# hpcaitech/Open-Sora

Measured on NVIDIA H100. Metric: denoise-steps/sec STDiT3-XL/2 64x32x32 bf16, higher is better.
Workload: dtype bf16

## Files before the change

### open-sora_b200/csrc/attn_sm90.cu

```cuda
#include <stdlib.h>

#include "common.cuh"
#include "stage.cuh"
#include "tiles.cuh"

namespace osb {

constexpr int kAttnThreads = 256;
constexpr int kKeyBlock = 64;

template <int D>
struct FlashState {
  static constexpr int DP = HeadTileCfg<D>::DP;
  uint32_t q[DP / 16][4];
  float o[DP / 8][4];
  float m[2], l[2];
};

template <int D>
__device__ __forceinline__ void flash_load_q(FlashState<D>& f, uint32_t sq, uint32_t chunk_bytes) {
  using Cfg = HeadTileCfg<D>;
  const int lane = threadIdx.x & 31, warp = threadIdx.x >> 5;
  const int row = warp * 16 + (lane & 15);
#pragma unroll
  for (int kk = 0; kk < Cfg::DP / 16; ++kk)
    ldsm_x4(sq + tile_unit_off<Cfg::MAIN>(row, 2 * kk + (lane >> 4), chunk_bytes), f.q[kk][0], f.q[kk][1], f.q[kk][2], f.q[kk][3]);
#pragma unroll
  for (int j = 0; j < Cfg::DP / 8; ++j) f.o[j][0] = f.o[j][1] = f.o[j][2] = f.o[j][3] = 0.f;
  f.m[0] = f.m[1] = -INFINITY;
  f.l[0] = f.l[1] = 0.f;
}

template <int D, bool kBias = false>
__device__ __forceinline__ void flash_block(FlashState<D>& f, uint32_t sk, uint32_t sv, uint32_t chunk_bytes, int krow0,
                                            int n16, int key0, const int (&lo)[2], const int (&hi)[2], float sc,
                                            const float* bias = nullptr, int boff0 = 0, int boff1 = 0, float bscale = 0.f) {
  using Cfg = HeadTileCfg<D>;
  constexpr int NB = kKeyBlock / 8;
  const int lane = threadIdx.x & 31;
  float s[NB][4];
#pragma unroll
  for (int g = 0; g < kKeyBlock / 16; ++g) {
    s[2 * g][0] = s[2 * g][1] = s[2 * g][2] = s[2 * g][3] = 0.f;
    s[2 * g + 1][0] = s[2 * g + 1][1] = s[2 * g + 1][2] = s[2 * g + 1][3] = 0.f;
    if (g >= n16) continue;
    const int krow = krow0 + g * 16 + (lane & 7) + ((lane >> 4) << 3);
#pragma unroll
    for (int kk = 0; kk < Cfg::DP / 16; ++kk) {
      uint32_t b0, b1, b2, b3;
      ldsm_x4(sk + tile_unit_off<Cfg::MAIN>(krow, 2 * kk + ((lane >> 3) & 1), chunk_bytes), b0, b1, b2, b3);
      mma_bf16_16816(s[2 * g], f.q[kk], b0, b1);
      mma_bf16_16816(s[2 * g + 1], f.q[kk], b2, b3);
    }
  }
  float mx[2] = {-INFINITY, -INFINITY};
#pragma unroll
  for (int j = 0; j < NB; ++j) {
// ... 19 lines not shown
  }
#pragma unroll
  for (int j = 0; j < Cfg::DP / 8; ++j) {
    f.o[j][0] *= alpha[0]; f.o[j][1] *= alpha[0];
    f.o[j][2] *= alpha[1]; f.o[j][3] *= alpha[1];
  }
#pragma unroll
  for (int j = 0; j < NB; ++j) {
#pragma unroll
    for (int e = 0; e < 4; ++e) {
      s[j][e] = fast_exp2(fmaf(s[j][e], sc, -ms[e >> 1]));
      f.l[e >> 1] += s[j][e];
    }
  }
#pragma unroll
  for (int g = 0; g < kKeyBlock / 16; ++g) {
    if (g >= n16) continue;
    const uint32_t a[4] = {pack_bf16x2(s[2 * g][0], s[2 * g][1]), pack_bf16x2(s[2 * g][2], s[2 * g][3]),
                           pack_bf16x2(s[2 * g + 1][0], s[2 * g + 1][1]), pack_bf16x2(s[2 * g + 1][2], s[2 * g + 1][3])};
    const int vrow = krow0 + g * 16 + (lane & 7) + (((lane >> 3) & 1) << 3);
#pragma unroll
    for (int dg = 0; dg < Cfg::DP / 16; ++dg) {
      uint32_t b0, b1, b2, b3;
      ldsm_x4_t(sv + tile_unit_off<Cfg::MAIN>(vrow, 2 * dg + (lane >> 4), chunk_bytes), b0, b1, b2, b3);
      mma_bf16_16816(f.o[2 * dg], a, b0, b1);
      mma_bf16_16816(f.o[2 * dg + 1], a, b2, b3);
    }
  }
}

template <int D>
__device__ __forceinline__ void flash_store(FlashState<D>& f, __nv_bfloat16* dst0, __nv_bfloat16* dst1) {
  const int lane = threadIdx.x & 31;
  float inv[2];
#pragma unroll
  for (int i = 0; i < 2; ++i) {
    float l = f.l[i];
    l += __shfl_xor_sync(0xffffffffu, l, 1);
    l += __shfl_xor_sync(0xffffffffu, l, 2);
    inv[i] = l > 0.f ? 1.0f / l : 0.f;
  }
#pragma unroll
  for (int j = 0; j < D / 8; ++j) {
    const int c = 8 * j + 2 * (lane & 3);
    if (dst0) *reinterpret_cast<uint32_t*>(dst0 + c) = pack_bf16x2(f.o[j][0] * inv[0], f.o[j][1] * inv[0]);
    if (dst1) *reinterpret_cast<uint32_t*>(dst1 + c) = pack_bf16x2(f.o[j][2] * inv[1], f.o[j][3] * inv[1]);
  }
}

struct TileAttnParams {
  const uint8_t* q; const uint8_t* k; const uint8_t* v;
  int64_t q_head_stride, kv_head_stride;
  TileMap qmap;
  int32_t q_tile_bytes, q_slot_bytes;
  int32_t kv_tile_bytes, kv_slot_bytes;
  int32_t BK, nkb, Lk;
  int64_t num_seqs, num_sets;
  const int32_t* kv_lens;
  __nv_bfloat16* out;
  int64_t out_ld;
  float scale_log2;
  RowScatter out_sc;
};

template <int D>
__global__ void __launch_bounds__(kAttnThreads, 1) attn_tiles_kernel(const TileAttnParams p) {
  extern __shared__ __align__(1024) uint8_t smem[];
  const uint32_t s0 = smem_u32(smem);
  const uint32_t sQ = s0;
  auto sK = [&](int st) { return s0 + (uint32_t)(p.q_slot_bytes + st * 2 * p.kv_slot_bytes); };
  auto sV = [&](int st) { return sK(st) + (uint32_t)p.kv_slot_bytes; };
  const uint32_t bar = s0 + (uint32_t)(p.q_slot_bytes + 4 * p.kv_slot_bytes);
  const uint32_t q_full = bar;
  auto kv_full = [&](int st) { return bar + 8u + 8u * st; };

  const int tid = threadIdx.x, lane = tid & 31, warp = tid >> 5;
  const int64_t qtile = blockIdx.x;
  const int head = blockIdx.y;
  const int64_t set = qtile / p.qmap.tps;
  const int qt = (int)(qtile - set * p.qmap.tps);

  int keys = p.qmap.G > 1 ? p.qmap.G * p.Lk : p.Lk;
  if (p.qmap.G == 1 && p.kv_lens) { const int l = __ldg(p.kv_lens + set); keys = l < keys ? (l < 0 ? 0 : l) : keys; }
  const int nkt = (keys + p.BK - 1) / p.BK;

  if (tid == 0) {
    mbar_init(q_full, 1);
    mbar_init(kv_full(0), 1);
    mbar_init(kv_full(1), 1);
    fence_barrier_init();
  }
  __syncthreads();
  pdl_wait();
  const uint8_t* kbase = p.k + (int64_t)head * p.kv_head_stride + set * p.nkb * (int64_t)p.kv_tile_bytes;
  const uint8_t* vbase = p.v + (int64_t)head * p.kv_head_stride + set * p.nkb * (int64_t)p.kv_tile_bytes;
  if (tid == 0) {
    mbar_expect_tx(q_full, (uint32_t)p.q_tile_bytes);
    bulk_load_1d(sQ, p.q + (int64_t)head * p.q_head_stride + qtile * p.q_tile_bytes, (uint32_t)p.q_tile_bytes, q_full);
    for (int st = 0; st < 2 && st < nkt; ++st) {
      mbar_expect_tx(kv_full(st), 2u * (uint32_t)p.kv_tile_bytes);
      bulk_load_1d(sK(st), kbase + (int64_t)st * p.kv_tile_bytes, (uint32_t)p.kv_tile_bytes, kv_full(st));
      bulk_load_1d(sV(st), vbase + (int64_t)st * p.kv_tile_bytes, (uint32_t)p.kv_tile_bytes, kv_full(st));
    }
  }

  int64_t seq[2];
  int pos[2], lo[2], hi[2];
  bool valid[2];
#pragma unroll
  for (int i = 0; i < 2; ++i) {
    const int r = warp * 16 + (lane >> 2) + 8 * i;
    lo[i] = hi[i] = 0;
    if (p.qmap.G > 1) {
      const int g = r / p.qmap.L;
      pos[i] = r - g * p.qmap.L;
      seq[i] = set * p.qmap.G + g;
      valid[i] = g < p.qmap.G && seq[i] < p.num_seqs;
      if (valid[i]) { lo[i] = g * p.Lk; hi[i] = lo[i] + p.Lk; }
    } else {
      pos[i] = qt * p.qmap.TR + r;
      seq[i] = set;
      valid[i] = r < p.qmap.TR && pos[i] < p.qmap.L;
      if (valid[i]) hi[i] = keys;
    }
  }

  FlashState<D> f;
  mbar_wait(q_full, 0);
  flash_load_q<D>(f, sQ, (uint32_t)p.qmap.TR * 128u);
  const float sc = p.scale_log2;
  for (int kb = 0; kb < nkt; ++kb) {
    const int st = kb & 1;
    mbar_wait(kv_full(st), (uint32_t)(kb >> 1) & 1u);
    for (int k0 = 0; k0 < p.BK; k0 += kKeyBlock) {
      int n = keys - (kb * p.BK + k0);
      const int cap = p.BK - k0 < kKeyBlock ? p.BK - k0 : kKeyBlock;
      n = n > cap ? cap : n;
      if (n <= 0) break;
      const int lo_b[2] = {lo[0], lo[1]}, hi_b[2] = {hi[0], hi[1]};
      flash_block<D>(f, sK(st), sV(st), (uint32_t)p.BK * 128u, k0, (n + 15) >> 4, kb * p.BK + k0, lo_b, hi_b, sc);
    }
    __syncthreads();
    if (tid == 0 && kb + 2 < nkt) {
      mbar_expect_tx(kv_full(st), 2u * (uint32_t)p.kv_tile_bytes);
      bulk_load_1d(sK(st), kbase + (int64_t)(kb + 2) * p.kv_tile_bytes, (uint32_t)p.kv_tile_bytes, kv_full(st));
      bulk_load_1d(sV(st), vbase + (int64_t)(kb + 2) * p.kv_tile_bytes, (uint32_t)p.kv_tile_bytes, kv_full(st));
    }
  }
  pdl_launch_dependents();

  __nv_bfloat16* dst[2] = {nullptr, nullptr};
#pragma unroll
  for (int i = 0; i < 2; ++i) {
    if (!valid[i]) continue;
    int64_t orow = row_of_token(p.qmap, seq[i], pos[i]);
    __nv_bfloat16* obase = p.out;
    if (p.out_sc.mode != 0) {
      int peer;
      scatter_row(p.out_sc, orow, peer, orow);
      obase = static_cast<__nv_bfloat16*>(scatter_base(p.out_sc, peer));
    }
    dst[i] = obase + orow * p.out_ld + (int64_t)head * D;
  }
  flash_store<D>(f, dst[0], dst[1]);
}

template <int D>
static int attn_tiles_launch(TileAttnParams& p, int H, cudaStream_t stream) {
  using Cfg = HeadTileCfg<D>;
  p.q_tile_bytes = p.qmap.TR * Cfg::ROW_BYTES;
  p.q_slot_bytes = 128 * Cfg::ROW_BYTES;
  p.kv_tile_bytes = p.BK * Cfg::ROW_BYTES;
  p.kv_slot_bytes = (p.kv_tile_bytes + 127) / 128 * 128;
  const int smem = p.q_slot_bytes + 4 * p.kv_slot_bytes + 64;
  const int64_t qtiles = p.num_sets * p.qmap.tps;
  if (qtiles >= (1ll << 31) || H > 65535) { set_error("osb_attn_tiles: problem too large (%lld query tiles)", (long long)qtiles); return OSB_ERR_UNSUPPORTED; }
  cudaLaunchAttribute attr[2];
  cudaLaunchConfig_t cfg = launch_config(dim3((unsigned)qtiles, (unsigned)H), dim3(kAttnThreads), smem, stream, attr);
  OSB_CHECK_CUDA(cudaLaunchKernelEx(&cfg, attn_tiles_kernel<D>, p));
  count_launch();
  return OSB_OK;
}

struct AttnParams {
  const __nv_bfloat16* q; const __nv_bfloat16* k; const __nv_bfloat16* v; __nv_bfloat16* out;
  int64_t q_ld, k_ld, v_ld, out_ld;
  int64_t num_seqs, seqs_per_batch;
  int64_t q_bs, q_ss, q_ts, k_bs, k_ss, k_ts;
  int32_t Lq, Lk;
  const int32_t* kv_lens;
  const __nv_bfloat16* qw; const __nv_bfloat16* kw;
  const __nv_bfloat16* qw2; const __nv_bfloat16* kw2;
  int32_t norm_split;
  float eps;
  const float* cos; const float* sin;
  int32_t rope_half;
  float scale_log2;
  int32_t G;
  int32_t tiles_per_seq;
  const float* bias;
  int64_t bias_hs;
  float scale;
};

template <int D>
__device__ __forceinline__ void stage_row(uint4 (&raw)[HeadTileCfg<D>::U], bool norm, float eps, const __nv_bfloat16* w,
                                          const float* cosr, const float* sinr, bool rope_half, uint8_t* tile,
                                          uint32_t chunk_bytes, int row) {
  using Cfg = HeadTileCfg<D>;
  constexpr int U = Cfg::U;
  norm_rope_row<D, U>(raw, norm, eps, w, cosr, sinr, rope_half);
#pragma unroll
  for (int u = 0; u < Cfg::UP; ++u)
    *reinterpret_cast<uint4*>(tile + tile_unit_off<Cfg::MAIN>(row, u, chunk_bytes)) = u < U ? raw[u] : make_uint4(0, 0, 0, 0);
}

template <int D, bool kBias>
__global__ void __launch_bounds__(kAttnThreads, 1) attn_short_kernel(const AttnParams p) {
  using Cfg = HeadTileCfg<D>;
  constexpr int U = Cfg::U;
  extern __shared__ __align__(1024) uint8_t smem[];
  uint8_t* sQ = smem;
  uint8_t* sK = smem + 128 * Cfg::ROW_BYTES;
  uint8_t* sV = sK + kKeyBlock * Cfg::ROW_BYTES;
  const int tid = threadIdx.x, lane = tid & 31, warp = tid >> 5;
  const int64_t unit = blockIdx.x;
  const int h = blockIdx.y;

  int64_t seq0;
  int qt = 0;
  if (p.G > 1) seq0 = unit * p.G;
// ... 71 lines not shown
      const int slot = k0 + s;
      const int kg = slot / p.Lk, ktok = slot - kg * p.Lk;
      const int64_t kseq = seq0 + kg;
      const bool ok = slot < nkeys && kseq < p.num_seqs;
      int64_t krow = 0;
      if (ok) krow = row_of(kseq, ktok, p.k_bs, p.k_ss, p.k_ts);
      uint4 t[U];
      {
        const uint4* ks = reinterpret_cast<const uint4*>(p.k + krow * p.k_ld + (int64_t)h * D);
#pragma unroll
        for (int u = 0; u < U; ++u) t[u] = ok ? __ldg(ks + u) : make_uint4(0, 0, 0, 0);
        const __nv_bfloat16* w = (p.kw2 != nullptr && ktok >= p.norm_split) ? p.kw2 : p.kw;
        const bool rope = ok && p.cos != nullptr;
        stage_row<D>(t, ok && p.kw != nullptr, p.eps, w, rope ? p.cos + (int64_t)ktok * (D / 2) : nullptr,
                     rope ? p.sin + (int64_t)ktok * (D / 2) : nullptr, p.rope_half, sK, kKeyBlock * 128u, s);
      }
      {
        const uint4* vs = reinterpret_cast<const uint4*>(p.v + krow * p.v_ld + (int64_t)h * D);
#pragma unroll
        for (int u = 0; u < U; ++u) t[u] = ok ? __ldg(vs + u) : make_uint4(0, 0, 0, 0);
        stage_row<D>(t, false, 0.f, nullptr, nullptr, nullptr, false, sV, kKeyBlock * 128u, s);
      }
    }
    __syncthreads();
    const int n = nkeys - k0 < kKeyBlock ? nkeys - k0 : kKeyBlock;
    if constexpr (kBias)
      flash_block<D, true>(f, smem_u32(sK), smem_u32(sV), kKeyBlock * 128u, 0, (n + 15) >> 4, k0, lo, hi, sc, bh, boff[0],
                           boff[1], p.scale);
    else
      flash_block<D>(f, smem_u32(sK), smem_u32(sV), kKeyBlock * 128u, 0, (n + 15) >> 4, k0, lo, hi, sc);
    __syncthreads();
  }
  pdl_launch_dependents();
  flash_store<D>(f, dst[0], dst[1]);
}

template <int D, bool kBias = false>
static int attn_short_launch(const AttnParams& p, int64_t units, int H, cudaStream_t stream) {
  using Cfg = HeadTileCfg<D>;
  const int smem = (128 + 2 * kKeyBlock) * Cfg::ROW_BYTES;
  cudaLaunchAttribute attr[2];
  cudaLaunchConfig_t cfg = launch_config(dim3((unsigned)units, (unsigned)H), dim3(kAttnThreads), smem, stream, attr);
  OSB_CHECK_CUDA(cudaLaunchKernelEx(&cfg, attn_short_kernel<D, kBias>, p));
  count_launch();
  return OSB_OK;
}

int attn_init() {
  constexpr int kMax = 200 * 1024;
  OSB_CHECK_CUDA(cudaFuncSetAttribute(attn_short_kernel<64, false>, cudaFuncAttributeMaxDynamicSharedMemorySize, kMax));
  OSB_CHECK_CUDA(cudaFuncSetAttribute(attn_short_kernel<72, false>, cudaFuncAttributeMaxDynamicSharedMemorySize, kMax));
  OSB_CHECK_CUDA(cudaFuncSetAttribute(attn_short_kernel<128, false>, cudaFuncAttributeMaxDynamicSharedMemorySize, kMax));
  OSB_CHECK_CUDA(cudaFuncSetAttribute(attn_short_kernel<64, true>, cudaFuncAttributeMaxDynamicSharedMemorySize, kMax));
  OSB_CHECK_CUDA(cudaFuncSetAttribute(attn_tiles_kernel<64>, cudaFuncAttributeMaxDynamicSharedMemorySize, kMax));
  OSB_CHECK_CUDA(cudaFuncSetAttribute(attn_tiles_kernel<72>, cudaFuncAttributeMaxDynamicSharedMemorySize, kMax));
  OSB_CHECK_CUDA(cudaFuncSetAttribute(attn_tiles_kernel<128>, cudaFuncAttributeMaxDynamicSharedMemorySize, kMax));
  return OSB_OK;
}

}

extern "C" int64_t osb_head_tiles_per_head(const osb_tile_map* m, int64_t rows) {
  if (m == nullptr || m->L <= 0 || m->tile_rows <= 0) return -1;
  const int64_t seqs = rows / m->L;
  if (m->G > 1) return (seqs + m->G - 1) / m->G;
  return seqs * m->tps;
}

extern "C" int osb_attn_tiles(const osb_attn_tiles_args* a, void* stream) {
  using namespace osb;
  if (!initialised()) { set_error("osb_init() has not been called"); return OSB_ERR_NOT_INIT; }
  OSB_REQUIRE(a != nullptr, "osb_attn_tiles: null args");
  OSB_REQUIRE(a->q_tiles && a->k_tiles && a->v_tiles && (a->out || a->out_scatter), "osb_attn_tiles: null tensor");
  const int D = a->head_dim;
  OSB_REQUIRE(D == 64 || D == 72 || D == 128, "osb_attn_tiles: head_dim %d not built (64, 72, 128)", D);
  const osb_tile_map& m = a->q_map;
  OSB_REQUIRE(m.mode == 0 || m.mode == 1, "osb_attn_tiles: unknown tile map mode %d", m.mode);
  OSB_REQUIRE(m.L > 0 && m.G >= 1 && m.tile_rows > 0 && m.tile_rows <= 128 && m.tile_rows % 8 == 0,
              "osb_attn_tiles: bad q tile map (L %d G %d rows %d)", m.L, m.G, m.tile_rows);
  OSB_REQUIRE(m.G == 1 ? (m.tps == (m.L + m.tile_rows - 1) / m.tile_rows) : (m.G * m.L <= m.tile_rows && m.tps == 1),
              "osb_attn_tiles: q tile map inconsistent (L %d G %d tps %d rows %d)", m.L, m.G, m.tps, m.tile_rows);
  OSB_REQUIRE(m.mode == 0 || (m.S > 0 && m.T == m.L), "osb_attn_tiles: temporal map needs S > 0 and T == L");
  OSB_REQUIRE(a->kv_tile_rows >= 16 && a->kv_tile_rows <= 128 && a->kv_tile_rows % 16 == 0,
              "osb_attn_tiles: key tiles must have 16..128 rows in multiples of 16, got %d", a->kv_tile_rows);
  OSB_REQUIRE(a->Lk > 0 && a->kv_tiles_per_set >= 1 && (int64_t)a->kv_tiles_per_set * a->kv_tile_rows >= (int64_t)(m.G > 1 ? m.G : 1) * a->Lk,
              "osb_attn_tiles: %d key tiles of %d rows cannot hold %d keys", a->kv_tiles_per_set, a->kv_tile_rows, a->Lk);
  OSB_REQUIRE(m.G == 1 || (a->kv_tiles_per_set == 1), "osb_attn_tiles: packed sequences use one key tile per set");
  OSB_REQUIRE(a->num_seqs > 0 && a->num_heads > 0, "osb_attn_tiles: empty problem");
  OSB_REQUIRE(a->out_ld % 8 == 0 && (reinterpret_cast<uintptr_t>(a->out) & 15) == 0, "osb_attn_tiles: out must be 16-byte aligned");
  OSB_REQUIRE(((reinterpret_cast<uintptr_t>(a->q_tiles) | reinterpret_cast<uintptr_t>(a->k_tiles) | reinterpret_cast<uintptr_t>(a->v_tiles)) & 15) == 0 &&
              a->q_head_stride % 16 == 0 && a->kv_head_stride % 16 == 0, "osb_attn_tiles: tile buffers must be 16-byte aligned");

  TileAttnParams p = {};
  p.q = static_cast<const uint8_t*>(a->q_tiles);
  p.k = static_cast<const uint8_t*>(a->k_tiles);
  p.v = static_cast<const uint8_t*>(a->v_tiles);
  p.q_head_stride = a->q_head_stride; p.kv_head_stride = a->kv_head_stride;
  p.qmap.mode = m.mode; p.qmap.L = m.L; p.qmap.S = m.S; p.qmap.T = m.T; p.qmap.G = m.G; p.qmap.tps = m.tps; p.qmap.TR = m.tile_rows;
  p.BK = a->kv_tile_rows; p.nkb = a->kv_tiles_per_set; p.Lk = a->Lk;
  p.num_seqs = a->num_seqs;
  p.num_sets = m.G > 1 ? (a->num_seqs + m.G - 1) / m.G : a->num_seqs;
  p.kv_lens = a->kv_lens;
  p.out = static_cast<__nv_bfloat16*>(a->out);
  p.out_ld = a->out_ld;
  p.scale_log2 = a->softmax_scale * 1.4426950408889634f;
  {
    const int64_t out_rows = a->num_seqs * m.L;
    const int rc = make_row_scatter(&p.out_sc, a->out_scatter, out_rows, "osb_attn_tiles");
    if (rc) return rc;
// ... 83 lines not shown
```

### open-sora_b200/csrc/wgmma.cuh

```cuda
#pragma once

#include <stdint.h>

namespace osb {

template <int N>
struct Wgmma;

template <>
struct Wgmma<64> {
  static constexpr int kRegs = 32;
  __device__ __forceinline__ static void mma(float (&d)[32], uint64_t da, uint64_t db, uint32_t accumulate) {
    asm volatile(
        "{\n\t.reg .pred p;\n\tsetp.ne.b32 p, %34, 0;\n\t"
        "wgmma.mma_async.sync.aligned.m64n64k16.f32.bf16.bf16 "
        "{%0, %1, %2, %3, %4, %5, %6, %7, %8, %9, %10, %11, %12, %13, %14, %15, %16, %17, %18, %19, %20, %21, %22, %23, %24, %25, %26, %27, %28, %29, %30, %31}, "
        "%32, %33, p, 1, 1, 0, 0;\n\t}\n"
        : "+f"(d[0]), "+f"(d[1]), "+f"(d[2]), "+f"(d[3]), "+f"(d[4]), "+f"(d[5]), "+f"(d[6]), "+f"(d[7]),
        "+f"(d[8]), "+f"(d[9]), "+f"(d[10]), "+f"(d[11]), "+f"(d[12]), "+f"(d[13]), "+f"(d[14]), "+f"(d[15]),
        "+f"(d[16]), "+f"(d[17]), "+f"(d[18]), "+f"(d[19]), "+f"(d[20]), "+f"(d[21]), "+f"(d[22]), "+f"(d[23]),
        "+f"(d[24]), "+f"(d[25]), "+f"(d[26]), "+f"(d[27]), "+f"(d[28]), "+f"(d[29]), "+f"(d[30]), "+f"(d[31])
        : "l"(da), "l"(db), "r"(accumulate));
  }
};
// ... 45 lines not shown
struct Wgmma<192> {
  static constexpr int kRegs = 96;
  __device__ __forceinline__ static void mma(float (&d)[96], uint64_t da, uint64_t db, uint32_t accumulate) {
    asm volatile(
        "{\n\t.reg .pred p;\n\tsetp.ne.b32 p, %98, 0;\n\t"
        "wgmma.mma_async.sync.aligned.m64n192k16.f32.bf16.bf16 "
        "{%0, %1, %2, %3, %4, %5, %6, %7, %8, %9, %10, %11, %12, %13, %14, %15, %16, %17, %18, %19, %20, %21, %22, %23, %24, %25, %26, %27, %28, %29, %30, %31, %32, %33, %34, %35, %36, %37, %38, %39, %40, %41, %42, %43, %44, %45, %46, %47, %48, %49, %50, %51, %52, %53, %54, %55, %56, %57, %58, %59, %60, %61, %62, %63, %64, %65, %66, %67, %68, %69, %70, %71, %72, %73, %74, %75, %76, %77, %78, %79, %80, %81, %82, %83, %84, %85, %86, %87, %88, %89, %90, %91, %92, %93, %94, %95}, "
        "%96, %97, p, 1, 1, 0, 0;\n\t}\n"
        : "+f"(d[0]), "+f"(d[1]), "+f"(d[2]), "+f"(d[3]), "+f"(d[4]), "+f"(d[5]), "+f"(d[6]), "+f"(d[7]),
        "+f"(d[8]), "+f"(d[9]), "+f"(d[10]), "+f"(d[11]), "+f"(d[12]), "+f"(d[13]), "+f"(d[14]), "+f"(d[15]),
        "+f"(d[16]), "+f"(d[17]), "+f"(d[18]), "+f"(d[19]), "+f"(d[20]), "+f"(d[21]), "+f"(d[22]), "+f"(d[23]),
        "+f"(d[24]), "+f"(d[25]), "+f"(d[26]), "+f"(d[27]), "+f"(d[28]), "+f"(d[29]), "+f"(d[30]), "+f"(d[31]),
        "+f"(d[32]), "+f"(d[33]), "+f"(d[34]), "+f"(d[35]), "+f"(d[36]), "+f"(d[37]), "+f"(d[38]), "+f"(d[39]),
        "+f"(d[40]), "+f"(d[41]), "+f"(d[42]), "+f"(d[43]), "+f"(d[44]), "+f"(d[45]), "+f"(d[46]), "+f"(d[47]),
        "+f"(d[48]), "+f"(d[49]), "+f"(d[50]), "+f"(d[51]), "+f"(d[52]), "+f"(d[53]), "+f"(d[54]), "+f"(d[55]),
        "+f"(d[56]), "+f"(d[57]), "+f"(d[58]), "+f"(d[59]), "+f"(d[60]), "+f"(d[61]), "+f"(d[62]), "+f"(d[63]),
        "+f"(d[64]), "+f"(d[65]), "+f"(d[66]), "+f"(d[67]), "+f"(d[68]), "+f"(d[69]), "+f"(d[70]), "+f"(d[71]),
        "+f"(d[72]), "+f"(d[73]), "+f"(d[74]), "+f"(d[75]), "+f"(d[76]), "+f"(d[77]), "+f"(d[78]), "+f"(d[79]),
        "+f"(d[80]), "+f"(d[81]), "+f"(d[82]), "+f"(d[83]), "+f"(d[84]), "+f"(d[85]), "+f"(d[86]), "+f"(d[87]),
        "+f"(d[88]), "+f"(d[89]), "+f"(d[90]), "+f"(d[91]), "+f"(d[92]), "+f"(d[93]), "+f"(d[94]), "+f"(d[95])
        : "l"(da), "l"(db), "r"(accumulate));
  }
};

template <>
struct Wgmma<256> {
  static constexpr int kRegs = 128;
  __device__ __forceinline__ static void mma(float (&d)[128], uint64_t da, uint64_t db, uint32_t accumulate) {
    asm volatile(
        "{\n\t.reg .pred p;\n\tsetp.ne.b32 p, %130, 0;\n\t"
        "wgmma.mma_async.sync.aligned.m64n256k16.f32.bf16.bf16 "
        "{%0, %1, %2, %3, %4, %5, %6, %7, %8, %9, %10, %11, %12, %13, %14, %15, %16, %17, %18, %19, %20, %21, %22, %23, %24, %25, %26, %27, %28, %29, %30, %31, %32, %33, %34, %35, %36, %37, %38, %39, %40, %41, %42, %43, %44, %45, %46, %47, %48, %49, %50, %51, %52, %53, %54, %55, %56, %57, %58, %59, %60, %61, %62, %63, %64, %65, %66, %67, %68, %69, %70, %71, %72, %73, %74, %75, %76, %77, %78, %79, %80, %81, %82, %83, %84, %85, %86, %87, %88, %89, %90, %91, %92, %93, %94, %95, %96, %97, %98, %99, %100, %101, %102, %103, %104, %105, %106, %107, %108, %109, %110, %111, %112, %113, %114, %115, %116, %117, %118, %119, %120, %121, %122, %123, %124, %125, %126, %127}, "
        "%128, %129, p, 1, 1, 0, 0;\n\t}\n"
        : "+f"(d[0]), "+f"(d[1]), "+f"(d[2]), "+f"(d[3]), "+f"(d[4]), "+f"(d[5]), "+f"(d[6]), "+f"(d[7]),
        "+f"(d[8]), "+f"(d[9]), "+f"(d[10]), "+f"(d[11]), "+f"(d[12]), "+f"(d[13]), "+f"(d[14]), "+f"(d[15]),
        "+f"(d[16]), "+f"(d[17]), "+f"(d[18]), "+f"(d[19]), "+f"(d[20]), "+f"(d[21]), "+f"(d[22]), "+f"(d[23]),
        "+f"(d[24]), "+f"(d[25]), "+f"(d[26]), "+f"(d[27]), "+f"(d[28]), "+f"(d[29]), "+f"(d[30]), "+f"(d[31]),
        "+f"(d[32]), "+f"(d[33]), "+f"(d[34]), "+f"(d[35]), "+f"(d[36]), "+f"(d[37]), "+f"(d[38]), "+f"(d[39]),
        "+f"(d[40]), "+f"(d[41]), "+f"(d[42]), "+f"(d[43]), "+f"(d[44]), "+f"(d[45]), "+f"(d[46]), "+f"(d[47]),
        "+f"(d[48]), "+f"(d[49]), "+f"(d[50]), "+f"(d[51]), "+f"(d[52]), "+f"(d[53]), "+f"(d[54]), "+f"(d[55]),
        "+f"(d[56]), "+f"(d[57]), "+f"(d[58]), "+f"(d[59]), "+f"(d[60]), "+f"(d[61]), "+f"(d[62]), "+f"(d[63]),
        "+f"(d[64]), "+f"(d[65]), "+f"(d[66]), "+f"(d[67]), "+f"(d[68]), "+f"(d[69]), "+f"(d[70]), "+f"(d[71]),
        "+f"(d[72]), "+f"(d[73]), "+f"(d[74]), "+f"(d[75]), "+f"(d[76]), "+f"(d[77]), "+f"(d[78]), "+f"(d[79]),
        "+f"(d[80]), "+f"(d[81]), "+f"(d[82]), "+f"(d[83]), "+f"(d[84]), "+f"(d[85]), "+f"(d[86]), "+f"(d[87]),
        "+f"(d[88]), "+f"(d[89]), "+f"(d[90]), "+f"(d[91]), "+f"(d[92]), "+f"(d[93]), "+f"(d[94]), "+f"(d[95]),
        "+f"(d[96]), "+f"(d[97]), "+f"(d[98]), "+f"(d[99]), "+f"(d[100]), "+f"(d[101]), "+f"(d[102]), "+f"(d[103]),
        "+f"(d[104]), "+f"(d[105]), "+f"(d[106]), "+f"(d[107]), "+f"(d[108]), "+f"(d[109]), "+f"(d[110]), "+f"(d[111]),
        "+f"(d[112]), "+f"(d[113]), "+f"(d[114]), "+f"(d[115]), "+f"(d[116]), "+f"(d[117]), "+f"(d[118]), "+f"(d[119]),
        "+f"(d[120]), "+f"(d[121]), "+f"(d[122]), "+f"(d[123]), "+f"(d[124]), "+f"(d[125]), "+f"(d[126]), "+f"(d[127])
        : "l"(da), "l"(db), "r"(accumulate));
  }
};

template <int N>
struct WgmmaFp8;
template <>
struct WgmmaFp8<64> {
  __device__ __forceinline__ static void mma(float (&d)[32], uint64_t da, uint64_t db, uint32_t accumulate) {
    asm volatile(
        "{\n\t.reg .pred p;\n\tsetp.ne.b32 p, %34, 0;\n\t"
        "wgmma.mma_async.sync.aligned.m64n64k32.f32.e4m3.e4m3 "
        "{%0, %1, %2, %3, %4, %5, %6, %7, %8, %9, %10, %11, %12, %13, %14, %15, %16, %17, %18, %19, %20, %21, %22, %23, %24, %25, %26, %27, %28, %29, %30, %31}, "
        "%32, %33, p, 1, 1;\n\t}\n"
        : "+f"(d[0]), "+f"(d[1]), "+f"(d[2]), "+f"(d[3]), "+f"(d[4]), "+f"(d[5]), "+f"(d[6]), "+f"(d[7]),
        "+f"(d[8]), "+f"(d[9]), "+f"(d[10]), "+f"(d[11]), "+f"(d[12]), "+f"(d[13]), "+f"(d[14]), "+f"(d[15]),
        "+f"(d[16]), "+f"(d[17]), "+f"(d[18]), "+f"(d[19]), "+f"(d[20]), "+f"(d[21]), "+f"(d[22]), "+f"(d[23]),
        "+f"(d[24]), "+f"(d[25]), "+f"(d[26]), "+f"(d[27]), "+f"(d[28]), "+f"(d[29]), "+f"(d[30]), "+f"(d[31])
        : "l"(da), "l"(db), "r"(accumulate));
  }
};
template <>
struct WgmmaFp8<128> {
  __device__ __forceinline__ static void mma(float (&d)[64], uint64_t da, uint64_t db, uint32_t accumulate) {
    asm volatile(
        "{\n\t.reg .pred p;\n\tsetp.ne.b32 p, %66, 0;\n\t"
        "wgmma.mma_async.sync.aligned.m64n128k32.f32.e4m3.e4m3 "
        "{%0, %1, %2, %3, %4, %5, %6, %7, %8, %9, %10, %11, %12, %13, %14, %15, %16, %17, %18, %19, %20, %21, %22, %23, %24, %25, %26, %27, %28, %29, %30, %31, %32, %33, %34, %35, %36, %37, %38, %39, %40, %41, %42, %43, %44, %45, %46, %47, %48, %49, %50, %51, %52, %53, %54, %55, %56, %57, %58, %59, %60, %61, %62, %63}, "
        "%64, %65, p, 1, 1;\n\t}\n"
        : "+f"(d[0]), "+f"(d[1]), "+f"(d[2]), "+f"(d[3]), "+f"(d[4]), "+f"(d[5]), "+f"(d[6]), "+f"(d[7]),
        "+f"(d[8]), "+f"(d[9]), "+f"(d[10]), "+f"(d[11]), "+f"(d[12]), "+f"(d[13]), "+f"(d[14]), "+f"(d[15]),
        "+f"(d[16]), "+f"(d[17]), "+f"(d[18]), "+f"(d[19]), "+f"(d[20]), "+f"(d[21]), "+f"(d[22]), "+f"(d[23]),
        "+f"(d[24]), "+f"(d[25]), "+f"(d[26]), "+f"(d[27]), "+f"(d[28]), "+f"(d[29]), "+f"(d[30]), "+f"(d[31]),
        "+f"(d[32]), "+f"(d[33]), "+f"(d[34]), "+f"(d[35]), "+f"(d[36]), "+f"(d[37]), "+f"(d[38]), "+f"(d[39]),
        "+f"(d[40]), "+f"(d[41]), "+f"(d[42]), "+f"(d[43]), "+f"(d[44]), "+f"(d[45]), "+f"(d[46]), "+f"(d[47]),
        "+f"(d[48]), "+f"(d[49]), "+f"(d[50]), "+f"(d[51]), "+f"(d[52]), "+f"(d[53]), "+f"(d[54]), "+f"(d[55]),
        "+f"(d[56]), "+f"(d[57]), "+f"(d[58]), "+f"(d[59]), "+f"(d[60]), "+f"(d[61]), "+f"(d[62]), "+f"(d[63])
        : "l"(da), "l"(db), "r"(accumulate));
  }
};
template <>
struct WgmmaFp8<192> {
  __device__ __forceinline__ static void mma(float (&d)[96], uint64_t da, uint64_t db, uint32_t accumulate) {
    asm volatile(
        "{\n\t.reg .pred p;\n\tsetp.ne.b32 p, %98, 0;\n\t"
        "wgmma.mma_async.sync.aligned.m64n192k32.f32.e4m3.e4m3 "
        "{%0, %1, %2, %3, %4, %5, %6, %7, %8, %9, %10, %11, %12, %13, %14, %15, %16, %17, %18, %19, %20, %21, %22, %23, %24, %25, %26, %27, %28, %29, %30, %31, %32, %33, %34, %35, %36, %37, %38, %39, %40, %41, %42, %43, %44, %45, %46, %47, %48, %49, %50, %51, %52, %53, %54, %55, %56, %57, %58, %59, %60, %61, %62, %63, %64, %65, %66, %67, %68, %69, %70, %71, %72, %73, %74, %75, %76, %77, %78, %79, %80, %81, %82, %83, %84, %85, %86, %87, %88, %89, %90, %91, %92, %93, %94, %95}, "
        "%96, %97, p, 1, 1;\n\t}\n"
        : "+f"(d[0]), "+f"(d[1]), "+f"(d[2]), "+f"(d[3]), "+f"(d[4]), "+f"(d[5]), "+f"(d[6]), "+f"(d[7]),
        "+f"(d[8]), "+f"(d[9]), "+f"(d[10]), "+f"(d[11]), "+f"(d[12]), "+f"(d[13]), "+f"(d[14]), "+f"(d[15]),
        "+f"(d[16]), "+f"(d[17]), "+f"(d[18]), "+f"(d[19]), "+f"(d[20]), "+f"(d[21]), "+f"(d[22]), "+f"(d[23]),
        "+f"(d[24]), "+f"(d[25]), "+f"(d[26]), "+f"(d[27]), "+f"(d[28]), "+f"(d[29]), "+f"(d[30]), "+f"(d[31]),
        "+f"(d[32]), "+f"(d[33]), "+f"(d[34]), "+f"(d[35]), "+f"(d[36]), "+f"(d[37]), "+f"(d[38]), "+f"(d[39]),
        "+f"(d[40]), "+f"(d[41]), "+f"(d[42]), "+f"(d[43]), "+f"(d[44]), "+f"(d[45]), "+f"(d[46]), "+f"(d[47]),
        "+f"(d[48]), "+f"(d[49]), "+f"(d[50]), "+f"(d[51]), "+f"(d[52]), "+f"(d[53]), "+f"(d[54]), "+f"(d[55]),
        "+f"(d[56]), "+f"(d[57]), "+f"(d[58]), "+f"(d[59]), "+f"(d[60]), "+f"(d[61]), "+f"(d[62]), "+f"(d[63]),
        "+f"(d[64]), "+f"(d[65]), "+f"(d[66]), "+f"(d[67]), "+f"(d[68]), "+f"(d[69]), "+f"(d[70]), "+f"(d[71]),
// ... 94 lines not shown
```

Before: 10.71.

## Rewrite tiled attention as persistent warp-specialized WGMMA kernel with KV reuse

Replaces the mma.sync flash-attention tile kernel with a persistent kernel that has one producer warpgroup issuing bulk loads into a multi-stage mbarrier ring and two consumer warpgroups running WGMMA for QK^T and PV. Q is double-buffered across work items. K/V tiles stay resident when consecutive query tiles share the same head/set and fit in the stage ring. The aim is higher tensor-core throughput, overlap of loads with compute, less redundant KV traffic and fewer CTA launches. Risks include correctness of descriptors and layouts for the 72-dim tail, register pressure under setmaxnreg, and load imbalance from the static persistent split.

```diff
diff --git a/open-sora_b200/csrc/attn_sm90.cu b/open-sora_b200/csrc/attn_sm90.cu
--- a/open-sora_b200/csrc/attn_sm90.cu
+++ b/open-sora_b200/csrc/attn_sm90.cu
@@ -3,6 +3,7 @@
 #include "common.cuh"
 #include "stage.cuh"
 #include "tiles.cuh"
+#include "wgmma.cuh"
 
 namespace osb {
 
@@ -128,10 +129,10 @@
   const uint8_t* q; const uint8_t* k; const uint8_t* v;
   int64_t q_head_stride, kv_head_stride;
   TileMap qmap;
-  int32_t q_tile_bytes, q_slot_bytes;
-  int32_t kv_tile_bytes, kv_slot_bytes;
+  int32_t q_tile_bytes, kv_tile_bytes;
   int32_t BK, nkb, Lk;
   int64_t num_seqs, num_sets;
+  int64_t items;
   const int32_t* kv_lens;
   __nv_bfloat16* out;
   int64_t out_ld;
@@ -140,119 +141,252 @@
 };
 
 template <int D>
-__global__ void __launch_bounds__(kAttnThreads, 1) attn_tiles_kernel(const TileAttnParams p) {
-  extern __shared__ __align__(1024) uint8_t smem[];
-  const uint32_t s0 = smem_u32(smem);
-  const uint32_t sQ = s0;
-  auto sK = [&](int st) { return s0 + (uint32_t)(p.q_slot_bytes + st * 2 * p.kv_slot_bytes); };
-  auto sV = [&](int st) { return sK(st) + (uint32_t)p.kv_slot_bytes; };
-  const uint32_t bar = s0 + (uint32_t)(p.q_slot_bytes + 4 * p.kv_slot_bytes);
-  const uint32_t q_full = bar;
-  auto kv_full = [&](int st) { return bar + 8u + 8u * st; };
-
-  const int tid = threadIdx.x, lane = tid & 31, warp = tid >> 5;
-  const int64_t qtile = blockIdx.x;
-  const int head = blockIdx.y;
-  const int64_t set = qtile / p.qmap.tps;
-  const int qt = (int)(qtile - set * p.qmap.tps);
-
+struct TileAttnSmem {
+  static constexpr int kSlot = 128 * HeadTileCfg<D>::ROW_BYTES;
+  static constexpr int kStages = D == 128 ? 2 : (D == 72 ? 4 : 5);
+  static constexpr int kData = 2 * kSlot + kStages * 2 * kSlot;
+  static constexpr int kBytes = 1024 + kData + 8 * (4 + 2 * kStages);
+  static_assert(kBytes <= 227 * 1024 && 2 * kBytes > 228 * 1024, "one resident CTA per SM");
+};
+
+constexpr int kTileAttnThreads = 384;
+
+__device__ __forceinline__ int tile_set_keys(const TileAttnParams& p, int64_t set) {
   int keys = p.qmap.G > 1 ? p.qmap.G * p.Lk : p.Lk;
   if (p.qmap.G == 1 && p.kv_lens) { const int l = __ldg(p.kv_lens + set); keys = l < keys ? (l < 0 ? 0 : l) : keys; }
-  const int nkt = (keys + p.BK - 1) / p.BK;
-
-  if (tid == 0) {
-    mbar_init(q_full, 1);
-    mbar_init(kv_full(0), 1);
-    mbar_init(kv_full(1), 1);
+  return keys;
+}
+
+template <int D>
+__global__ void __launch_bounds__(kTileAttnThreads, 1) attn_tiles_kernel(const TileAttnParams p) {
+  using Cfg = HeadTileCfg<D>;
+  using Sm = TileAttnSmem<D>;
+  constexpr int MAIN = Cfg::MAIN, TAIL = Cfg::TAIL, STAGES = Sm::kStages;
+  extern __shared__ uint8_t smem_raw[];
+  const uint32_t base = (smem_u32(smem_raw) + 1023u) & ~1023u;
+  auto sQ = [&](int b) { return base + (uint32_t)(b * Sm::kSlot); };
+  auto sK = [&](int s) { return base + (uint32_t)((2 + 2 * s) * Sm::kSlot); };
+  auto sV = [&](int s) { return sK(s) + (uint32_t)Sm::kSlot; };
+  const uint32_t bar = base + (uint32_t)Sm::kData;
+  auto q_full = [&](int b) { return bar + 8u * b; };
+  auto q_empty = [&](int b) { return bar + 16u + 8u * b; };
+  auto full_bar = [&](int s) { return bar + 32u + 8u * s; };
+  auto empty_bar = [&](int s) { return bar + 32u + 8u * (STAGES + s); };
+
+  const int wg = threadIdx.x >> 7, tid_wg = threadIdx.x & 127;
+  const int64_t begin = (int64_t)blockIdx.x * p.items / gridDim.x, end = (int64_t)(blockIdx.x + 1) * p.items / gridDim.x;
+  const int tps = p.qmap.tps;
+
+  {
+    uint4* z = reinterpret_cast<uint4*>(smem_raw + (base - smem_u32(smem_raw)));
+    for (int i = threadIdx.x; i < Sm::kData / 16; i += kTileAttnThreads) z[i] = make_uint4(0, 0, 0, 0);
+  }
+  fence_proxy_async_smem();
+  if (threadIdx.x == 0) {
+    for (int b = 0; b < 2; ++b) { mbar_init(q_full(b), 1); mbar_init(q_empty(b), 2); }
+    for (int s = 0; s < STAGES; ++s) { mbar_init(full_bar(s), 1); mbar_init(empty_bar(s), 2); }
     fence_barrier_init();
   }
   __syncthreads();
   pdl_wait();
-  const uint8_t* kbase = p.k + (int64_t)head * p.kv_head_stride + set * p.nkb * (int64_t)p.kv_tile_bytes;
-  const uint8_t* vbase = p.v + (int64_t)head * p.kv_head_stride + set * p.nkb * (int64_t)p.kv_tile_bytes;
-  if (tid == 0) {
-    mbar_expect_tx(q_full, (uint32_t)p.q_tile_bytes);
-    bulk_load_1d(sQ, p.q + (int64_t)head * p.q_head_stride + qtile * p.q_tile_bytes, (uint32_t)p.q_tile_bytes, q_full);
-    for (int st = 0; st < 2 && st < nkt; ++st) {
-      mbar_expect_tx(kv_full(st), 2u * (uint32_t)p.kv_tile_bytes);
-      bulk_load_1d(sK(st), kbase + (int64_t)st * p.kv_tile_bytes, (uint32_t)p.kv_tile_bytes, kv_full(st));
-      bulk_load_1d(sV(st), vbase + (int64_t)st * p.kv_tile_bytes, (uint32_t)p.kv_tile_bytes, kv_full(st));
-    }
-  }
-
-  int64_t seq[2];
-  int pos[2], lo[2], hi[2];
-  bool valid[2];
-#pragma unroll
-  for (int i = 0; i < 2; ++i) {
-    const int r = warp * 16 + (lane >> 2) + 8 * i;
-    lo[i] = hi[i] = 0;
-    if (p.qmap.G > 1) {
-      const int g = r / p.qmap.L;
-      pos[i] = r - g * p.qmap.L;
-      seq[i] = set * p.qmap.G + g;
-      valid[i] = g < p.qmap.G && seq[i] < p.num_seqs;
-      if (valid[i]) { lo[i] = g * p.Lk; hi[i] = lo[i] + p.Lk; }
-    } else {
-      pos[i] = qt * p.qmap.TR + r;
-      seq[i] = set;
-      valid[i] = r < p.qmap.TR && pos[i] < p.qmap.L;
-      if (valid[i]) hi[i] = keys;
-    }
-  }
-
-  FlashState<D> f;
-  mbar_wait(q_full, 0);
-  flash_load_q<D>(f, sQ, (uint32_t)p.qmap.TR * 128u);
+
+  if (wg == 0) {
+    asm volatile("setmaxnreg.dec.sync.aligned.u32 40;\n" ::: "memory");
+    if (tid_wg == 0) {
+      uint32_t kv_it = 0;
+      for (int64_t it = begin; it < end; ++it) {
+        const uint32_t n = (uint32_t)(it - begin);
+        const int64_t hs = it / tps, head = hs / p.num_sets, set = hs - head * p.num_sets;
+        const int qs = n & 1;
+        mbar_wait_notrace(q_empty(qs), ((n >> 1) & 1u) ^ 1u);
+        mbar_expect_tx(q_full(qs), (uint32_t)p.q_tile_bytes);
+        bulk_load_1d(sQ(qs), p.q + head * p.q_head_stride + (it - head * p.num_sets * tps) * p.q_tile_bytes,
+                     (uint32_t)p.q_tile_bytes, q_full(qs));
+        const int nkt = (tile_set_keys(p, set) + p.BK - 1) / p.BK;
+        if (it > begin && (it - 1) / tps == hs && nkt <= STAGES) continue;
+        const int64_t off = head * p.kv_head_stride + set * p.nkb * (int64_t)p.kv_tile_bytes;
+        for (int t = 0; t < nkt; ++t, ++kv_it) {
+          const int s = (int)(kv_it % STAGES);
+          mbar_wait_notrace(empty_bar(s), ((kv_it / STAGES) & 1u) ^ 1u);
+          mbar_expect_tx(full_bar(s), 2u * (uint32_t)p.kv_tile_bytes);
+          bulk_load_1d(sK(s), p.k + off + (int64_t)t * p.kv_tile_bytes, (uint32_t)p.kv_tile_bytes, full_bar(s));
+          bulk_load_1d(sV(s), p.v + off + (int64_t)t * p.kv_tile_bytes, (uint32_t)p.kv_tile_bytes, full_bar(s));
+        }
+      }
+      pdl_launch_dependents();
+    }
+    return;
+  }
+
+  asm volatile("setmaxnreg.inc.sync.aligned.u32 232;\n" ::: "memory");
+  const int cw = wg - 1;
+  const int lane = tid_wg & 31, quad = lane & 3;
+  const int r_loc = cw * 64 + (tid_wg >> 5) * 16 + (lane >> 2);
   const float sc = p.scale_log2;
-  for (int kb = 0; kb < nkt; ++kb) {
-    const int st = kb & 1;
-    mbar_wait(kv_full(st), (uint32_t)(kb >> 1) & 1u);
-    for (int k0 = 0; k0 < p.BK; k0 += kKeyBlock) {
-      int n = keys - (kb * p.BK + k0);
-      const int cap = p.BK - k0 < kKeyBlock ? p.BK - k0 : kKeyBlock;
-      n = n > cap ? cap : n;
-      if (n <= 0) break;
-      const int lo_b[2] = {lo[0], lo[1]}, hi_b[2] = {hi[0], hi[1]};
-      flash_block<D>(f, sK(st), sV(st), (uint32_t)p.BK * 128u, k0, (n + 15) >> 4, kb * p.BK + k0, lo_b, hi_b, sc);
-    }
-    __syncthreads();
-    if (tid == 0 && kb + 2 < nkt) {
-      mbar_expect_tx(kv_full(st), 2u * (uint32_t)p.kv_tile_bytes);
-      bulk_load_1d(sK(st), kbase + (int64_t)(kb + 2) * p.kv_tile_bytes, (uint32_t)p.kv_tile_bytes, kv_full(st));
-      bulk_load_1d(sV(st), vbase + (int64_t)(kb + 2) * p.kv_tile_bytes, (uint32_t)p.kv_tile_bytes, kv_full(st));
-    }
-  }
-  pdl_launch_dependents();
-
-  __nv_bfloat16* dst[2] = {nullptr, nullptr};
-#pragma unroll
-  for (int i = 0; i < 2; ++i) {
-    if (!valid[i]) continue;
-    int64_t orow = row_of_token(p.qmap, seq[i], pos[i]);
-    __nv_bfloat16* obase = p.out;
-    if (p.out_sc.mode != 0) {
-      int peer;
-      scatter_row(p.out_sc, orow, peer, orow);
-      obase = static_cast<__nv_bfloat16*>(scatter_base(p.out_sc, peer));
-    }
-    dst[i] = obase + orow * p.out_ld + (int64_t)head * D;
-  }
-  flash_store<D>(f, dst[0], dst[1]);
+  float s[64], o[MAIN][32], ot[TAIL ? 8 : 1];
+#pragma unroll
+  for (int i = 0; i < 64; ++i) s[i] = 0.f;
+  uint32_t kv_it = 0, kv0 = 0;
+  for (int64_t it = begin; it < end; ++it) {
+    const uint32_t n = (uint32_t)(it - begin);
+    const int64_t hs = it / tps, head = hs / p.num_sets, set = hs - head * p.num_sets;
+    const int qt = (int)(it - hs * tps), qs = n & 1;
+    const int keys = tile_set_keys(p, set);
+    const int nkt = (keys + p.BK - 1) / p.BK;
+    if (!(it > begin && (it - 1) / tps == hs && nkt <= STAGES)) { kv0 = kv_it; kv_it += nkt; }
+    const bool keep = it + 1 < end && (it + 1) / tps == hs && nkt <= STAGES;
+
+    int64_t seq[2];
+    int pos[2], lo[2], hi[2];
+    bool valid[2];
+#pragma unroll
+    for (int hh = 0; hh < 2; ++hh) {
+      const int r = r_loc + 8 * hh;
+      lo[hh] = hi[hh] = 0;
+      if (p.qmap.G > 1) {
+        const int g = r / p.qmap.L;
+        pos[hh] = r - g * p.qmap.L;
+        seq[hh] = set * p.qmap.G + g;
+        valid[hh] = g < p.qmap.G && seq[hh] < p.num_seqs;
+        if (valid[hh]) { lo[hh] = g * p.Lk; hi[hh] = lo[hh] + p.Lk; }
+      } else {
+        pos[hh] = qt * p.qmap.TR + r;
+        seq[hh] = set;
+        valid[hh] = r < p.qmap.TR && pos[hh] < p.qmap.L;
+        if (valid[hh]) hi[hh] = keys;
+      }
+    }
+#pragma unroll
+    for (int c = 0; c < MAIN; ++c)
+#pragma unroll
+      for (int i = 0; i < 32; ++i) o[c][i] = 0.f;
+#pragma unroll
+    for (int i = 0; i < (TAIL ? 8 : 1); ++i) ot[i] = 0.f;
+    float m[2] = {-INFINITY, -INFINITY}, l[2] = {0.f, 0.f};
+
+    const uint32_t q_chunk = (uint32_t)p.qmap.TR * 128u, kv_chunk = (uint32_t)p.BK * 128u;
+    const uint32_t qa = sQ(qs) + (uint32_t)(cw * 64 * 128), qa_tail = sQ(qs) + MAIN * q_chunk + (uint32_t)(cw * 8 * 256);
+    mbar_wait_notrace(q_full(qs), (n >> 1) & 1u);
+    for (int t = 0; t < nkt; ++t) {
+      const uint32_t u = kv0 + (uint32_t)t;
+      const int st = (int)(u % STAGES);
+      mbar_wait_notrace(full_bar(st), (u / STAGES) & 1u);
+      const uint32_t ka = sK(st), va = sV(st);
+      wgmma_fence_regs(s);
+      wgmma_fence();
+#pragma unroll
+      for (int c = 0; c < MAIN; ++c)
+#pragma unroll
+        for (int k = 0; k < 4; ++k)
+          Wgmma<128>::mma(s, make_sw128_kmajor_desc(qa + c * q_chunk + 32u * k),
+                          make_sw128_kmajor_desc(ka + c * kv_chunk + 32u * k), (c | k) ? 1u : 0u);
+      if constexpr (TAIL != 0)
+        Wgmma<128>::mma(s, make_noswizzle_desc(qa_tail, 128u, 256u), make_noswizzle_desc(ka + MAIN * kv_chunk, 128u, 256u), 1u);
+      wgmma_commit();
+      wgmma_wait<0>();
+      wgmma_fence_regs(s);
+      if (t == nkt - 1 && tid_wg == 0) mbar_arrive(q_empty(qs));
+      const int slot0 = t * p.BK;
+      const int n16 = ((keys - slot0 < p.BK ? keys - slot0 : p.BK) + 15) >> 4;
+      float mx[2] = {-INFINITY, -INFINITY};
+#pragma unroll
+      for (int i = 0; i < 64; ++i) {
+        const int hh = (i >> 1) & 1;
+        const int col = 8 * (i >> 2) + 2 * quad + (i & 1), key = slot0 + col;
+        if (col >= p.BK || key < lo[hh] || key >= hi[hh]) s[i] = -INFINITY;
+        mx[hh] = fmaxf(mx[hh], s[i]);
+      }
+      float alpha[2], ms[2];
+#pragma unroll
+      for (int hh = 0; hh < 2; ++hh) {
+        mx[hh] = fmaxf(mx[hh], __shfl_xor_sync(0xffffffffu, mx[hh], 1));
+        mx[hh] = fmaxf(mx[hh], __shfl_xor_sync(0xffffffffu, mx[hh], 2));
+        const float mn = fmaxf(m[hh], mx[hh]);
+        alpha[hh] = (mn == -INFINITY) ? 1.f : fast_exp2((m[hh] - mn) * sc);
+        ms[hh] = (mn == -INFINITY) ? 0.f : mn * sc;
+        m[hh] = mn;
+        l[hh] *= alpha[hh];
+      }
+#pragma unroll
+      for (int c = 0; c < MAIN; ++c)
+#pragma unroll
+        for (int i = 0; i < 32; ++i) o[c][i] *= alpha[(i >> 1) & 1];
+      if constexpr (TAIL != 0) {
+#pragma unroll
+        for (int i = 0; i < 8; ++i) ot[i] *= alpha[(i >> 1) & 1];
+      }
+      uint32_t pa[8][4];
+#pragma unroll
+      for (int i = 0; i < 64; ++i) {
+        s[i] = (i >> 3) < n16 ? fast_exp2(fmaf(s[i], sc, -ms[(i >> 1) & 1])) : 0.f;
+        l[(i >> 1) & 1] += s[i];
+      }
+#pragma unroll
+      for (int g = 0; g < 8; ++g) {
+        pa[g][0] = pack_bf16x2(s[8 * g + 0], s[8 * g + 1]);
+        pa[g][1] = pack_bf16x2(s[8 * g + 2], s[8 * g + 3]);
+        pa[g][2] = pack_bf16x2(s[8 * g + 4], s[8 * g + 5]);
+        pa[g][3] = pack_bf16x2(s[8 * g + 6], s[8 * g + 7]);
+      }
+#pragma unroll
+      for (int c = 0; c < MAIN; ++c) wgmma_fence_regs(o[c]);
+      if constexpr (TAIL != 0) wgmma_fence_regs(ot);
+      wgmma_fence();
+#pragma unroll
+      for (int g = 0; g < 8; ++g) {
+#pragma unroll
+        for (int c = 0; c < MAIN; ++c)
+          WgmmaRegAT<64>::mma(o[c], pa[g], make_sw128_kmajor_desc(va + c * kv_chunk + 2048u * g), 1u);
+        if constexpr (TAIL != 0)
+          WgmmaRegAT<16>::mma(ot, pa[g], make_noswizzle_desc(va + MAIN * kv_chunk + 512u * g, 256u, 128u), 1u);
+      }
+      wgmma_commit();
+      wgmma_wait<0>();
+#pragma unroll
+      for (int c = 0; c < MAIN; ++c) wgmma_fence_regs(o[c]);
+      if constexpr (TAIL != 0) wgmma_fence_regs(ot);
+#pragma unroll
+      for (int g = 0; g < 8; ++g) fence_regs_u32(pa[g]);
+      if (!keep && tid_wg == 0) mbar_arrive(empty_bar(st));
+    }
+    if (nkt == 0 && tid_wg == 0) mbar_arrive(q_empty(qs));
+
+#pragma unroll
+    for (int hh = 0; hh < 2; ++hh) {
+      float lt = l[hh];
+      lt += __shfl_xor_sync(0xffffffffu, lt, 1);
+      lt += __shfl_xor_sync(0xffffffffu, lt, 2);
+      const float inv = lt > 0.f ? 1.0f / lt : 0.f;
+      if (!valid[hh]) continue;
+      int64_t orow = row_of_token(p.qmap, seq[hh], pos[hh]);
+      __nv_bfloat16* obase = p.out;
+      if (p.out_sc.mode != 0) {
+        int peer;
+        scatter_row(p.out_sc, orow, peer, orow);
+        obase = static_cast<__nv_bfloat16*>(scatter_base(p.out_sc, peer));
+      }
+      __nv_bfloat16* dst = obase + orow * p.out_ld + head * D + 2 * quad;
+#pragma unroll
+      for (int c = 0; c < MAIN; ++c)
+#pragma unroll
+        for (int j = 0; j < 8; ++j)
+          *reinterpret_cast<uint32_t*>(dst + 64 * c + 8 * j) = pack_bf16x2(o[c][4 * j + 2 * hh] * inv, o[c][4 * j + 2 * hh + 1] * inv);
+      if constexpr (TAIL != 0)
+        *reinterpret_cast<uint32_t*>(dst + 64 * MAIN) = pack_bf16x2(ot[2 * hh] * inv, ot[2 * hh + 1] * inv);
+    }
+  }
 }
 
 template <int D>
 static int attn_tiles_launch(TileAttnParams& p, int H, cudaStream_t stream) {
   using Cfg = HeadTileCfg<D>;
   p.q_tile_bytes = p.qmap.TR * Cfg::ROW_BYTES;
-  p.q_slot_bytes = 128 * Cfg::ROW_BYTES;
   p.kv_tile_bytes = p.BK * Cfg::ROW_BYTES;
-  p.kv_slot_bytes = (p.kv_tile_bytes + 127) / 128 * 128;
-  const int smem = p.q_slot_bytes + 4 * p.kv_slot_bytes + 64;
-  const int64_t qtiles = p.num_sets * p.qmap.tps;
-  if (qtiles >= (1ll << 31) || H > 65535) { set_error("osb_attn_tiles: problem too large (%lld query tiles)", (long long)qtiles); return OSB_ERR_UNSUPPORTED; }
+  p.items = (int64_t)H * p.num_sets * p.qmap.tps;
+  if (p.items >= (1ll << 31)) { set_error("osb_attn_tiles: problem too large (%lld work items)", (long long)p.items); return OSB_ERR_UNSUPPORTED; }
+  const int64_t grid = p.items < sm_count() ? p.items : sm_count();
   cudaLaunchAttribute attr[2];
-  cudaLaunchConfig_t cfg = launch_config(dim3((unsigned)qtiles, (unsigned)H), dim3(kAttnThreads), smem, stream, attr);
+  cudaLaunchConfig_t cfg = launch_config(dim3((unsigned)grid), dim3(kTileAttnThreads), TileAttnSmem<D>::kBytes, stream, attr);
   OSB_CHECK_CUDA(cudaLaunchKernelEx(&cfg, attn_tiles_kernel<D>, p));
   count_launch();
   return OSB_OK;
@@ -430,9 +564,9 @@
   OSB_CHECK_CUDA(cudaFuncSetAttribute(attn_short_kernel<72, false>, cudaFuncAttributeMaxDynamicSharedMemorySize, kMax));
   OSB_CHECK_CUDA(cudaFuncSetAttribute(attn_short_kernel<128, false>, cudaFuncAttributeMaxDynamicSharedMemorySize, kMax));
   OSB_CHECK_CUDA(cudaFuncSetAttribute(attn_short_kernel<64, true>, cudaFuncAttributeMaxDynamicSharedMemorySize, kMax));
-  OSB_CHECK_CUDA(cudaFuncSetAttribute(attn_tiles_kernel<64>, cudaFuncAttributeMaxDynamicSharedMemorySize, kMax));
-  OSB_CHECK_CUDA(cudaFuncSetAttribute(attn_tiles_kernel<72>, cudaFuncAttributeMaxDynamicSharedMemorySize, kMax));
-  OSB_CHECK_CUDA(cudaFuncSetAttribute(attn_tiles_kernel<128>, cudaFuncAttributeMaxDynamicSharedMemorySize, kMax));
+  OSB_CHECK_CUDA(cudaFuncSetAttribute(attn_tiles_kernel<64>, cudaFuncAttributeMaxDynamicSharedMemorySize, TileAttnSmem<64>::kBytes));
+  OSB_CHECK_CUDA(cudaFuncSetAttribute(attn_tiles_kernel<72>, cudaFuncAttributeMaxDynamicSharedMemorySize, TileAttnSmem<72>::kBytes));
+  OSB_CHECK_CUDA(cudaFuncSetAttribute(attn_tiles_kernel<128>, cudaFuncAttributeMaxDynamicSharedMemorySize, TileAttnSmem<128>::kBytes));
   return OSB_OK;
 }
 
diff --git a/open-sora_b200/csrc/wgmma.cuh b/open-sora_b200/csrc/wgmma.cuh
--- a/open-sora_b200/csrc/wgmma.cuh
+++ b/open-sora_b200/csrc/wgmma.cuh
@@ -121,6 +121,43 @@
   }
 };
 
+__device__ __forceinline__ uint64_t make_noswizzle_desc(uint32_t smem_addr, uint32_t lbo, uint32_t sbo) {
+  uint64_t d = 0;
+  d |= static_cast<uint64_t>((smem_addr & 0x3FFFF) >> 4);
+  d |= static_cast<uint64_t>(lbo >> 4) << 16;
+  d |= static_cast<uint64_t>(sbo >> 4) << 32;
+  return d;
+}
+
+template <int N>
+struct WgmmaRegAT;
+template <>
+struct WgmmaRegAT<64> {
+  __device__ __forceinline__ static void mma(float (&d)[32], const uint32_t (&a)[4], uint64_t db, uint32_t accumulate) {
+    asm volatile(
+        "{\n\t.reg .pred p;\n\tsetp.ne.b32 p, %37, 0;\n\t"
+        "wgmma.mma_async.sync.aligned.m64n64k16.f32.bf16.bf16 "
+        "{%0, %1, %2, %3, %4, %5, %6, %7, %8, %9, %10, %11, %12, %13, %14, %15, %16, %17, %18, %19, %20, %21, %22, %23, %24, %25, %26, %27, %28, %29, %30, %31}, "
+        "{%32, %33, %34, %35}, %36, p, 1, 1, 1;\n\t}\n"
+        : "+f"(d[0]), "+f"(d[1]), "+f"(d[2]), "+f"(d[3]), "+f"(d[4]), "+f"(d[5]), "+f"(d[6]), "+f"(d[7]),
+        "+f"(d[8]), "+f"(d[9]), "+f"(d[10]), "+f"(d[11]), "+f"(d[12]), "+f"(d[13]), "+f"(d[14]), "+f"(d[15]),
+        "+f"(d[16]), "+f"(d[17]), "+f"(d[18]), "+f"(d[19]), "+f"(d[20]), "+f"(d[21]), "+f"(d[22]), "+f"(d[23]),
+        "+f"(d[24]), "+f"(d[25]), "+f"(d[26]), "+f"(d[27]), "+f"(d[28]), "+f"(d[29]), "+f"(d[30]), "+f"(d[31])
+        : "r"(a[0]), "r"(a[1]), "r"(a[2]), "r"(a[3]), "l"(db), "r"(accumulate));
+  }
+};
+template <>
+struct WgmmaRegAT<16> {
+  __device__ __forceinline__ static void mma(float (&d)[8], const uint32_t (&a)[4], uint64_t db, uint32_t accumulate) {
+    asm volatile(
+        "{\n\t.reg .pred p;\n\tsetp.ne.b32 p, %13, 0;\n\t"
+        "wgmma.mma_async.sync.aligned.m64n16k16.f32.bf16.bf16 "
+        "{%0, %1, %2, %3, %4, %5, %6, %7}, {%8, %9, %10, %11}, %12, p, 1, 1, 1;\n\t}\n"
+        : "+f"(d[0]), "+f"(d[1]), "+f"(d[2]), "+f"(d[3]), "+f"(d[4]), "+f"(d[5]), "+f"(d[6]), "+f"(d[7])
+        : "r"(a[0]), "r"(a[1]), "r"(a[2]), "r"(a[3]), "l"(db), "r"(accumulate));
+  }
+};
+
 template <int N>
 struct WgmmaFp8;
 template <>
```

New measurement: 11.29, median of 6. 5.3% higher.
